# lcp29/trimesh-ray-optix

Hardware: AMD Instinct MI355X
Metric: Mrays/s closest-hit, 1M-tri mesh, 1024^2 ray batch (higher is better)
Workload: dtype f32; 1 GPU; C5(i): icosphere(8)+displacement seed 0, 1310720 tris; 1024x1024 pinhole rays per GPU; intersects_closest (stream_compaction=False); rays_per_gpu=1048576, rays_total=1048576, triangles=1310720, parallelism=ray-sharded x1, BVH replicated, warmup_steps_done=352, bvh_depth=30, bvh_bytes=104857568

## Files before the change

### trimesh-ray-optix_amd/csrc/kernels_direct.inc

```
template <bool C, bool DEEP = false> struct tr_word { typedef uint64_t T; };
template <> struct tr_word<true, false> { typedef uint32_t T; };

constexpr bool TR_STREAM_QN = true;
template <int Q> constexpr bool TR_STREAM_COLD = Q != TR_Q_CLOSEST;
template <int Q, int K, bool STATS, bool COMPACT = false, bool UNI = false, bool DEEP = false>
__device__ __forceinline__ void wave_traverse(const tr_bvh_view& b, tr_ray& r, bool go,
                                              tr_result& res, tr_topk<K>& top, tr_counters* cnt,
                                              const tr_ring ring) {
    tr_result_init(res);
    if (Q == TR_Q_LOCATION) top.init();
    typedef typename tr_word<COMPACT, DEEP>::T W;
    tr_state_t<W> fs;
    tr_state_init(fs);
    if (!go) fs.node = -1;
    while (!tr_done(fs)) {
        tr_fused_step<Q, K, STATS, COMPACT, W, UNI, true>(b, r, fs, res, top, cnt, ring);
        TR_CONVERGE();
        tr_fused_step<Q, K, STATS, COMPACT, W, UNI, false>(b, r, fs, res, top, cnt, ring);
        TR_CONVERGE();
    }
}

constexpr uint32_t TR_STEAL_EVERY = 3u;
constexpr uint32_t TR_STEAL_EARLY = 4u;
constexpr int TR_STEAL_IDLE = 1;
__device__ __forceinline__ int lane_rank(unsigned long long mask) {
    return (int)__builtin_amdgcn_mbcnt_hi((unsigned)(mask >> 32), __builtin_amdgcn_mbcnt_lo((unsigned)mask, 0u));
}

template <int Q, bool STATS, bool COMPACT, bool DEEP = false, bool QN = false>
__device__ __forceinline__ bool wave_traverse_steal(const tr_bvh_view& b, tr_ray& r, bool go,
                                                    tr_result& res, tr_counters* cnt,
                                                    const tr_ring ring, int32_t* wl, int lane,
                                                    uint32_t steal_min, bool& lost) {
    constexpr bool PLAIN = QN;
    typedef typename std::conditional<PLAIN, tr_plaina_w, typename tr_word<COMPACT, DEEP>::T>::type W;
    lost = false;
    tr_result_init(res);
    tr_topk<1> top;
    tr_state_t<W> fs;
    const tr_aring ar = tr_aring_of(ring);
    (void)ar;
    if constexpr (PLAIN) tr_state_init(fs, tr_addr_start(ring));
    else tr_state_init(fs);
    if (!go) fs.node = -1;
    auto trip_step = [&](auto test_tag) {
        constexpr bool TEST = decltype(test_tag)::value;
        if (!tr_done(fs)) tr_fused_step<Q, 1, STATS, COMPACT, W, false, TEST, QN>(b, r, fs, res, top, cnt, ring);
    };
    int owner = lane;
    bool split = false;
    uint32_t trip = 0;
    if (steal_min & 0x8000u) {
        steal_min &= 0x7fffu;
        const unsigned long long act = __ballot(go);
        if (act != 0ull) {
            const int l0 = (int)__builtin_ctzll(act);
            const float ax = __shfl(r.dx, l0), ay = __shfl(r.dy, l0), az = __shfl(r.dz, l0);
            const float bx = __shfl(r.ox, l0) - r.ox, by = __shfl(r.oy, l0) - r.oy, bz = __shfl(r.oz, l0) - r.oz;
            const float dd = ax * r.dx + ay * r.dy + az * r.dz;
            const float n0 = ax * ax + ay * ay + az * az, n1 = r.dx * r.dx + r.dy * r.dy + r.dz * r.dz;
            const float ex = 65535.f * b.frame.scale[0], ey = 65535.f * b.frame.scale[1], ez = 65535.f * b.frame.scale[2];
            const bool alike = dd > 0.f && dd * dd >= 0.998f * n0 * n1 && bx * bx + by * by + bz * bz <= 1e-4f * (ex * ex + ey * ey + ez * ez);
            if (4 * __popcll(__ballot(go && alike)) < 3 * __popcll(act) && steal_min > TR_STEAL_EARLY) steal_min = TR_STEAL_EARLY;
        }
    }
    typedef __attribute__((address_space(3))) volatile int32_t lds_i32;
    typedef __attribute__((address_space(3))) volatile unsigned long long lds_u64;
    lds_i32* const lw = (lds_i32*)wl;
    lds_i32* const list = lw;
    lds_i32* const xnode = lw + 64;
    lds_i32* const xdepth = lw + 128;
    int32_t* const xflags = wl + 128;
    if constexpr (PLAIN) xdepth[lane] = 0;
    constexpr int ACC = 192;
    int32_t* sum = wl + ACC;
    unsigned long long* keys = reinterpret_cast<unsigned long long*>(wl + ACC);
    lds_i32* const vsum = lw + ACC;
    lds_u64* const vkeys = (lds_u64*)(lw + ACC);
    lds_i32* const vslots = lw + ACC + 128;
    auto deposit = [&]() {
        if constexpr (PLAIN) {
            if (tr_addr_lost(fs.sa)) atomicOr(&xflags[owner], 0x100);
        }
        if (Q == TR_Q_COUNT) {
            if (res.count) atomicAdd(&sum[owner], res.count);
        } else if (Q == TR_Q_ANY) {
            if (res.best_face >= 0) vsum[owner] = 1;
        } else {
            const bool have = res.best_slot >= 0;
            const unsigned long long key = ((unsigned long long)(__float_as_uint(res.best_t) & 0x7fffffffu) << 32) |
                                           (unsigned)res.best_face;
            if (have) atomicMin(&keys[owner], key);
            __builtin_amdgcn_wave_barrier();
            if (have && vkeys[owner] == key) vslots[owner] = res.best_slot;
        }
    };
    for (;;) {
#pragma unroll 1
        for (uint32_t k = 0; k <= TR_STEAL_EVERY; k += 2) {
            trip_step(std::true_type{});
            TR_CONVERGE();
            trip_step(std::false_type{});
            TR_CONVERGE();
        }
        trip += (TR_STEAL_EVERY / 2u + 1u) * 2u;
        if (split) {
            if (Q == TR_Q_ANY) {
                if (res.best_face >= 0) vsum[owner] = 1;
                __builtin_amdgcn_wave_barrier();
                if (vsum[owner] != 0 && !tr_done(fs)) { fs.node = -1; fs.p0 = -1; fs.p1 = -1; fs.p2 = -1; }
            } else if (Q == TR_Q_CLOSEST || Q == TR_Q_FIRST) {
                const bool have = res.best_slot >= 0;
                const unsigned long long mine = ((unsigned long long)(__float_as_uint(res.best_t) & 0x7fffffffu) << 32) |
                                                (unsigned)(res.best_face < 0 ? 0x7fffffff : res.best_face);
                if (have) atomicMin(&keys[owner], mine);
                __builtin_amdgcn_wave_barrier();
                const unsigned long long k = vkeys[owner];
                if (have && k == mine) vslots[owner] = res.best_slot;
                if (k < mine) {
                    tr_set_best_t(res, __uint_as_float((unsigned)(k >> 32)));
                    res.best_face = (int32_t)(unsigned)k;
                    res.best_slot = -1;
                }
            }
        }
        const bool done = tr_done(fs);
        const unsigned long long idle = __ballot(done);
        if (idle == ~0ull) break;
        if (__popcll(idle) >= TR_STEAL_IDLE && trip >= steal_min) {
            uint32_t bot = 0;
            bool has_far;
            if constexpr (PLAIN) {
                bot = (uint32_t)xdepth[lane] & 0xffu;
                has_far = tr_addr_can_give(ar, fs.sa, bot);
            } else {
                has_far = (fs.trail & fs.owned) != 0;
            }
            const bool can_give = !done && has_far;
            const unsigned long long donors = __ballot(can_give);
            const int ni = __popcll(idle), nd = __popcll(donors);
            const int np = ni < nd ? ni : nd;
            if (np > 0) {
                if (!split) {
                    if (Q == TR_Q_COUNT || Q == TR_Q_ANY) vsum[lane] = 0;
                    else vkeys[lane] = ~0ull;
                    split = true;
                    __builtin_amdgcn_wave_barrier();
                }
                const int drank = lane_rank(donors), irank = lane_rank(idle);
                const bool give = can_give && drank < np;
                int gnode = 0, gdepth = 0;
                (void)gdepth;
                if constexpr (PLAIN) {
                    if (give) {
                        gnode = tr_addr_give(ar, fs.sa, bot);
                        list[drank] = lane; xnode[lane] = gnode;
                        atomicAdd(&xflags[lane], 1);
                    }
                } else if (give) {
                    uint32_t j;
                    gnode = tr_ring_get(ring, tr_bottom_slot<W>(fs.trail, fs.owned, j));
                    gdepth = (int32_t)(j + 1);
                    list[drank] = lane; xnode[lane] = gnode; xdepth[lane] = gdepth;
                    fs.trail &= ~(W(1) << j);
                }
                __builtin_amdgcn_wave_barrier();
                const bool take = done && irank < np;
                const int src = take ? list[irank] : lane;
                if (take) {
                    deposit();
                    tr_result_init(res);
                }
                r.ox = __shfl(r.ox, src); r.oy = __shfl(r.oy, src); r.oz = __shfl(r.oz, src);
                r.dx = __shfl(r.dx, src); r.dy = __shfl(r.dy, src); r.dz = __shfl(r.dz, src);
                r.ix = __shfl(r.ix, src); r.iy = __shfl(r.iy, src); r.iz = __shfl(r.iz, src);
                r.kd = __shfl(r.kd, src);
                r.sel_n = (uint32_t)__shfl((int)r.sel_n, src); r.sel_f = (uint32_t)__shfl((int)r.sel_f, src); r.sel_z = (uint32_t)__shfl((int)r.sel_z, src);
                if constexpr (QN) {
                    r.qax = __shfl(r.qax, src); r.qay = __shfl(r.qay, src); r.qaz = __shfl(r.qaz, src);
                    r.qnx = __shfl(r.qnx, src); r.qny = __shfl(r.qny, src); r.qnz = __shfl(r.qnz, src);
                    r.qfx = __shfl(r.qfx, src); r.qfy = __shfl(r.qfy, src); r.qfz = __shfl(r.qfz, src);
                    r.qaz2 = r.qaz;
                }
                const int own2 = __shfl(owner, src);
                const float bt = __shfl(res.best_t, src);
                if (take) {
                    owner = own2;
                    if constexpr (PLAIN) {
                        tr_state_init(fs, tr_addr_bottom(ar, fs.sa));
                        atomicAnd(&xflags[lane], 0x100);
                    } else {
                        tr_state_init(fs);
                        fs.depth = (uint32_t)xdepth[src];
                    }
                    fs.node = xnode[src];
                    tr_set_best_t(res, bt);
                }
                __builtin_amdgcn_wave_barrier();
            }
        }
    }
    if (split) {
        deposit();
        __builtin_amdgcn_wave_barrier();
        if (Q == TR_Q_COUNT) {
            res.count = vsum[lane];
        } else if (Q == TR_Q_ANY) {
            res.best_face = vsum[lane] ? 0 : -1;
        } else {
            const unsigned long long k = vkeys[lane];
            tr_result_init(res);
            if (k != ~0ull) {
                tr_set_best_t(res, __uint_as_float((unsigned)(k >> 32)));
                res.best_face = (int32_t)(unsigned)k;
                res.best_slot = vslots[lane];
            }
        }
        if constexpr (PLAIN) lost = (xdepth[lane] & 0x100) != 0;
    } else if constexpr (PLAIN) {
        lost = tr_addr_lost(fs.sa);
    }
    return split;
}

template <int Q, bool STATS, bool COMPACT = false, bool UNI = false, bool DEEP = false>
__device__ __forceinline__ void process_ray(const tr_bvh_view& b, const RayFetch& rf,
                                            const QueryOut& out, int64_t i, bool in_range,
                                            tr_counters* cnt, const tr_ring ring) {
    float o[3] = {0.f, 0.f, 0.f}, d[3] = {0.f, 0.f, 0.f};
    if (in_range) fetch_ray(rf, i, o, d);
    tr_ray r;
    const bool valid = tr_ray_setup_a(r, b.frame, o[0], o[1], o[2], d[0], d[1], d[2]) && in_range;
    tr_result res;
    if (Q == TR_Q_LOCATION) {
        tr_topk<0> top;
        top.ent = out.hits + (in_range ? i : 0) * out.cap;
        top.tris = b.tris;
        top.cap = out.cap;
        if (b.num_tris >= 2) {
            wave_traverse<Q, 0, STATS, COMPACT, UNI, DEEP>(b, r, valid, res, top, cnt, ring);
        } else {
            top.init();
            brute_one<Q>(b, r, valid, res);
            if (res.count) top.insert(res.best_t, res.best_face, 0);
        }
    } else {
        tr_topk<1> top;
        if (b.num_tris >= 2) wave_traverse<Q, 1, STATS, COMPACT, UNI, DEEP>(b, r, valid, res, top, cnt, ring);
        else brute_one<Q>(b, r, valid, res);
    }
    if (in_range) write_result<Q>(b, out, i, r, res);
}

template <int Q>
__device__ __attribute__((noinline)) tr_result retraverse_lost(const tr_node* nodes, const tr_link* links, const tr_tri* tris,
                                                               float b0, float b1, float b2, float s0, float s1, float s2,
                                                               float ox, float oy, float oz, float dx, float dy, float dz,
                                                               float best_t, int32_t best_face, int32_t best_slot) {
    tr_bvh_view v;
    v.nodes = nodes; v.links = links; v.tris = tris; v.num_tris = 2; v.qnodes = nullptr; v.frame_dev = nullptr;
    v.frame.base[0] = b0; v.frame.base[1] = b1; v.frame.base[2] = b2;
    v.frame.scale[0] = s0; v.frame.scale[1] = s1; v.frame.scale[2] = s2;
    tr_result res;
    res.best_t = best_t; res.best_face = best_face; res.best_slot = best_slot; res.count = 0;
    tr_ray r;
    if (tr_ray_setup_a(r, v.frame, ox, oy, oz, dx, dy, dz)) {
        tr_topk<1> top;
        tr_counters* nc = nullptr;
        tr_traverse_more<Q, 1, false>(v, r, res, top, nc);
    }
    return res;
}

template <int Q, bool STATS, bool COMPACT, bool DEEP = false, bool QN = false>
__device__ __forceinline__ void process_ray_steal(const tr_bvh_view& b, const RayFetch& rf,
                                                  const QueryOut& out, int64_t i, bool in_range,
                                                  tr_counters* cnt, const tr_ring ring, int32_t* wl,
                                                  uint32_t steal_min) {
    float o[3] = {0.f, 0.f, 0.f}, d[3] = {0.f, 0.f, 0.f};
    if (in_range) fetch_ray(rf, i, o, d);
    tr_ray r;
    const bool valid = tr_ray_setup_q(r, b.frame, o[0], o[1], o[2], d[0], d[1], d[2]) && in_range;
    tr_result res;
    bool split = false, lost = false;
    if (b.num_tris >= 2) split = wave_traverse_steal<Q, STATS, COMPACT, DEEP, QN>(b, r, valid, res, cnt, ring, wl, (int)(threadIdx.x & 63), steal_min, lost);
    else brute_one<Q>(b, r, valid, res);
    if (split && in_range) {
        fetch_ray(rf, i, o, d);
        tr_ray_setup_a(r, b.frame, o[0], o[1], o[2], d[0], d[1], d[2]);
    }
    if constexpr (QN) {
        lost = lost && valid;
        if (__builtin_expect(TR_WAVE_ANY(lost), 0)) {
            if (lost) {
                fetch_ray(rf, i, o, d);
                res = retraverse_lost<Q>(b.nodes, b.links, b.tris, b.frame.base[0], b.frame.base[1], b.frame.base[2],
                                         b.frame.scale[0], b.frame.scale[1], b.frame.scale[2], o[0], o[1], o[2], d[0], d[1], d[2],
                                         res.best_t, res.best_face, res.best_slot);
            }
        }
    }
    if (in_range) write_result<Q>(b, out, i, r, res);
}

template <int Q, int K, bool STATS, bool COMPACT, bool DEEP = false>
__device__ __forceinline__ void wave_traverse_unordered(const tr_bvh_view& b, tr_ray& r, bool go,
                                                        tr_result& res, tr_topk<K>& top, tr_counters* cnt,
                                                        const tr_ring ring, const tr_leafq lq, int leaf_min) {
    typedef typename tr_word<COMPACT, DEEP>::T W;
    tr_result_init(res);
    if (Q == TR_Q_LOCATION) top.init();
    tr_ustate_t<W> st;
    tr_ustate_init(st);
    if (!go) st.node = -1;
    for (;;) {
        const bool can_node = tr_ucan_node(st);
        const unsigned long long mn = __ballot(can_node), ml = __ballot(st.nq > 0);
        if ((mn | ml) == 0ull) break;
        const bool parked = st.node >= 0 && !can_node;
        const bool leaf_phase = mn == 0ull || __ballot(parked) != 0ull || (int)__popcll(ml) >= (int)leaf_min;
        tr_unord_step<Q, K, STATS, COMPACT, W>(b, r, can_node, leaf_phase, st, res, top, cnt, ring, lq);
        TR_CONVERGE();
    }
}

template <int Q, bool STATS, bool COMPACT, bool DEEP = false>
__device__ __forceinline__ int wave_count_unordered_steal(const tr_bvh_view& b, tr_ray& r, bool go, tr_counters* cnt,
                                                          const tr_ring ring, const tr_leafq lq, int leaf_min,
                                                          int lane, uint32_t steal_min) {
    typedef typename tr_word<COMPACT, DEEP>::T W;
    tr_result res;
    tr_result_init(res);
    tr_topk<1> top;
    tr_ustate_t<W> st;
    tr_ustate_init(st);
    if (!go) st.node = -1;
    int owner = lane;
    int acc = 0;
    uint32_t trip = 0;
    auto hand_in = [&](bool want) {
        unsigned long long m = __ballot(want && res.count != 0);
        while (m != 0ull) {
            const int t = (int)__builtin_ctzll(m);
            const int o = __builtin_amdgcn_readlane(owner, t), c = __builtin_amdgcn_readlane(res.count, t);
            if (lane == o) acc += c;
            m &= m - 1ull;
        }
        if (want) res.count = 0;
    };
    for (;;) {
        bool live = true;
#pragma unroll 1
        for (int k = 0; k < 4 && live; k++) {
            const bool can_node = tr_ucan_node(st);
            const unsigned long long mn = __ballot(can_node), ml = __ballot(st.nq > 0);
            live = (mn | ml) != 0ull;
            if (live) {
                const bool parked = st.node >= 0 && !can_node;
                const bool leaf_phase = mn == 0ull || __ballot(parked) != 0ull || (int)__popcll(ml) >= (int)leaf_min;
                tr_unord_step<Q, 1, STATS, COMPACT, W>(b, r, can_node, leaf_phase, st, res, top, cnt, ring, lq);
            }
            TR_CONVERGE();
        }
        trip += 4;
        const bool done = tr_udone(st);
        const unsigned long long idle = __ballot(done);
        if (idle == ~0ull) break;
        if (idle == 0ull) continue;
        const W cand = st.trail & st.owned;
        const bool can_give = !done && cand != 0 && trip >= steal_min;
        const unsigned long long donors = __ballot(can_give);
        const int ni = __popcll(idle), nd = __popcll(donors);
        const int np = ni < nd ? ni : nd;
        if (np == 0) continue;
        const int drank = lane_rank(donors), irank = lane_rank(idle);
        const bool give = can_give && drank < np;
        const bool take = done && irank < np;
        const unsigned long long givers = __ballot(give);
        const int tgt = give ? drank : 63 - lane_rank(~givers);
        const int list = __builtin_amdgcn_ds_permute(tgt << 2, lane);
        const int pick = __shfl(list, irank & 63);
        const int src = take ? pick : lane;
        int gnode = 0, gdepth = 0;
        if (give) {
            const uint32_t j = (uint32_t)__builtin_ctzll((unsigned long long)cand);
            gnode = tr_ring_get(ring, j & (TR_RING - 1));
            gdepth = (int)(j + 1);
            st.trail &= ~(W(1) << j);
            st.owned &= ~(W(1) << j);
        }
        if (take && owner == lane) { acc += res.count; res.count = 0; }
        hand_in(take && owner != lane);
        r.ox = __shfl(r.ox, src); r.oy = __shfl(r.oy, src); r.oz = __shfl(r.oz, src);
        r.dx = __shfl(r.dx, src); r.dy = __shfl(r.dy, src); r.dz = __shfl(r.dz, src);
        r.ix = __shfl(r.ix, src); r.iy = __shfl(r.iy, src); r.iz = __shfl(r.iz, src);
        r.kd = __shfl(r.kd, src);
        r.sel_n = (uint32_t)__shfl((int)r.sel_n, src); r.sel_f = (uint32_t)__shfl((int)r.sel_f, src); r.sel_z = (uint32_t)__shfl((int)r.sel_z, src);
        r.qax = __shfl(r.qax, src); r.qay = __shfl(r.qay, src); r.qaz = __shfl(r.qaz, src);
        r.qnx = __shfl(r.qnx, src); r.qny = __shfl(r.qny, src); r.qnz = __shfl(r.qnz, src);
        r.qfx = __shfl(r.qfx, src); r.qfy = __shfl(r.qfy, src); r.qfz = __shfl(r.qfz, src);
        r.qaz2 = r.qaz;
        const int own2 = __shfl(owner, src), n2 = __shfl(gnode, src), d2 = __shfl(gdepth, src);
        if (take) {
            owner = own2;
            tr_ustate_init(st);
            st.node = n2;
            st.depth = (uint32_t)d2;
// ... 384 lines not shown
```

### trimesh-ray-optix_amd/csrc/tr_bvh.h

```cpp
#pragma once
#include <type_traits>
#include "tr_math.h"
#include "../../include/triro_hip.h"

struct alignas(16) tr_f4 {
    float x, y, z, w;
};
struct alignas(16) tr_i4 {
    int32_t x, y, z, w;
};

struct alignas(64) tr_node {
    float box0[6];
    float box1[6];
    int32_t c0, c1;
    int32_t parent;
    int32_t sibling;
};
static_assert(sizeof(tr_node) == 64, "node must be 64 B");
TR_HD void tr_node_set_box(float* box, const float* lo, const float* hi) {
    box[0] = lo[0]; box[1] = lo[1]; box[2] = lo[2]; box[3] = hi[2]; box[4] = hi[0]; box[5] = hi[1];
}

struct alignas(8) tr_link {
// ... 492 lines not shown
    if (STATS) cnt->nodes++;
    float tn0, tf0, tn1, tf1;
    tr_node_slabs(r, n0, n1, n2, tn0, tf0, tn1, tf1);
    union { float f; int32_t i; } u0, u1, u2, u3;
    u0.f = n3.x; u1.f = n3.y; u2.f = n3.z; u3.f = n3.w;
    const int32_t c0 = u0.i, c1 = u1.i;
    int32_t parent = u2.i, sibling = u3.i;
    const float lim = tr_cull_limit<Q>(res);
    bool h0 = tr_slab_hit(tn0, tf0, lim);
    bool h1 = tr_slab_hit(tn1, tf1, lim);
    if (h0 && c0 < 0) { st.p0 = ~c0; h0 = false; }
    if (h1 && c1 < 0) { st.p1 = ~c1; h1 = false; }
    if (h0 | h1) {
        const bool both = h0 & h1;
        const bool swap = both ? (tn1 < tn0) : h1;
        if (both) {
            tr_push_far(ring, st.trail, st.owned, st.depth, swap ? c0 : c1);
            st.trail |= (1ull << st.depth);
        }
        st.node = swap ? c1 : c0;
        st.depth++;
    } else if (st.trail == 0) {
        st.node = -1;
    } else {
        uint32_t j = 0;
        int32_t far = -1;
        if (tr_pop_far(ring, st.trail, st.owned, j, far)) {
            st.node = far;
        } else {
            int32_t node = st.node;
            uint32_t depth = st.depth;
            while (depth > j + 1) {
                node = parent;
                const tr_link l = b.links[node];
                parent = l.parent; sibling = l.sibling;
                depth--;
                if (STATS) cnt->climbs++;
            }
            st.node = sibling;
        }
        st.depth = j + 1;
    }
}

template <int Q, int K, bool STATS>
TR_HD void tr_leaf_step(const tr_bvh_view& b, const tr_ray& r, tr_state& st, tr_result& res,
                        tr_topk<K>& top, tr_counters* cnt) {
    const int32_t q0 = st.p0, q1 = st.p1;
    tr_counters* nc = nullptr;
    const bool any1 = TR_WAVE_ANY(q1 >= 0);
    const tr_tri t0 = tr_load_tri<false>(b, q0 >= 0 ? q0 : 0, nc);
    tr_tri t1 = t0;
    if (any1) t1 = tr_load_tri<false>(b, q1 >= 0 ? q1 : 0, nc);
    if (STATS && q0 >= 0) cnt->tris++;
    bool fin = tr_fold_leaf<Q, K>(q0 >= 0, r, t0, q0, res, top, st.pe);
    fin = tr_drain_exact<Q, K>(b, r, st.pe, res, top) || fin;
    if (any1) {
        const bool live = q1 >= 0 && !fin;
        if (STATS && live) cnt->tris++;
        fin = tr_fold_leaf<Q, K>(live, r, t1, q1, res, top, st.pe) || fin;
        fin = tr_drain_exact<Q, K>(b, r, st.pe, res, top) || fin;
    }
    st.p0 = -1; st.p1 = -1;
    if (Q == TR_Q_ANY && fin) st.node = -1;
}

TR_HD void tr_qnode_slabs_contract(const tr_ray& r, const tr_qframe& f, const tr_i4& w0, const tr_i4& w1,
                                   float& tn0, float& tf0, float& tn1, float& tf1) {
    const uint32_t q0 = (uint32_t)w0.x, q1 = (uint32_t)w0.y, q2 = (uint32_t)w0.z, q3 = (uint32_t)w0.w;
    const uint32_t q4 = (uint32_t)w1.x, q5 = (uint32_t)w1.y;
    const float sx = f.scale[0], sy = f.scale[1], sz = f.scale[2], bx = f.base[0], by = f.base[1], bz = f.base[2];
    tr_slab(r, tr_qdecode(q0 & 0xffffu, sx, bx), tr_qdecode(q0 >> 16, sy, by), tr_qdecode(q1 & 0xffffu, sz, bz),
            tr_qdecode(q2 & 0xffffu, sx, bx), tr_qdecode(q2 >> 16, sy, by), tr_qdecode(q1 >> 16, sz, bz), tn0, tf0);
    tr_slab(r, tr_qdecode(q3 & 0xffffu, sx, bx), tr_qdecode(q3 >> 16, sy, by), tr_qdecode(q4 & 0xffffu, sz, bz),
            tr_qdecode(q5 & 0xffffu, sx, bx), tr_qdecode(q5 >> 16, sy, by), tr_qdecode(q4 >> 16, sz, bz), tn1, tf1);
}

TR_HD void tr_qnode_slabs(const tr_ray& r, const tr_qframe& f, const tr_i4& w0, const tr_i4& w1,
                          float& tn0, float& tf0, float& tn1, float& tf1) {
#if defined(__HIP_DEVICE_COMPILE__)
    const uint32_t q0 = (uint32_t)w0.x, q1 = (uint32_t)w0.y, q2 = (uint32_t)w0.z, q3 = (uint32_t)w0.w;
    const uint32_t q4 = (uint32_t)w1.x, q5 = (uint32_t)w1.y;
    typedef float tr_v2 __attribute__((ext_vector_type(2)));
    const tr_v2 axy = {r.qax, r.qay}, azz = {r.qaz, r.qaz2};
    const tr_v2 nxy = {r.qnx, r.qny}, fxy = {r.qfx, r.qfy}, bz = {r.qnz, r.qfz};
#define TR_UNPK(w) tr_v2{(float)((w) & 0xffffu), (float)((w) >> 16)}
    {
        const uint32_t pn = __builtin_amdgcn_perm(q2, q0, r.sel_n), pf = __builtin_amdgcn_perm(q2, q0, r.sel_f);
        const uint32_t zz = __builtin_amdgcn_perm(q1, q1, r.sel_z);
        const tr_v2 a = __builtin_elementwise_fma(TR_UNPK(pn), axy, nxy);
        const tr_v2 c = __builtin_elementwise_fma(TR_UNPK(pf), axy, fxy);
        const tr_v2 b = __builtin_elementwise_fma(TR_UNPK(zz), azz, bz);
        tn0 = fmaxf(fmaxf(a.x, a.y), b.x);
        tf0 = fminf(fminf(c.x, c.y), b.y);
    }
    {
        const uint32_t pn = __builtin_amdgcn_perm(q5, q3, r.sel_n), pf = __builtin_amdgcn_perm(q5, q3, r.sel_f);
        const uint32_t zz = __builtin_amdgcn_perm(q4, q4, r.sel_z);
        const tr_v2 a = __builtin_elementwise_fma(TR_UNPK(pn), axy, nxy);
        const tr_v2 c = __builtin_elementwise_fma(TR_UNPK(pf), axy, fxy);
        const tr_v2 b = __builtin_elementwise_fma(TR_UNPK(zz), azz, bz);
        tn1 = fmaxf(fmaxf(a.x, a.y), b.x);
        tf1 = fminf(fminf(c.x, c.y), b.y);
    }
#undef TR_UNPK
#else
    (void)f;
    const bool nx = r.ix < 0.f, ny = r.iy < 0.f, nz = r.iz < 0.f;
    const uint32_t q[6] = {(uint32_t)w0.x, (uint32_t)w0.y, (uint32_t)w0.z, (uint32_t)w0.w, (uint32_t)w1.x, (uint32_t)w1.y};
    float tn[2], tf[2];
    for (int c = 0; c < 2; c++) {
        const uint32_t lox = q[3 * c] & 0xffffu, loy = q[3 * c] >> 16, loz = q[3 * c + 1] & 0xffffu;
        const uint32_t hiz = q[3 * c + 1] >> 16, hix = q[3 * c + 2] & 0xffffu, hiy = q[3 * c + 2] >> 16;
        const float ax = fmaf((float)(nx ? hix : lox), r.qax, r.qnx), ay = fmaf((float)(ny ? hiy : loy), r.qay, r.qny);
        const float az = fmaf((float)(nz ? hiz : loz), r.qaz, r.qnz);
        const float cx = fmaf((float)(nx ? lox : hix), r.qax, r.qfx), cy = fmaf((float)(ny ? loy : hiy), r.qay, r.qfy);
        const float cz = fmaf((float)(nz ? loz : hiz), r.qaz, r.qfz);
        tn[c] = fmaxf(fmaxf(ax, ay), az);
        tf[c] = fminf(fminf(cx, cy), cz);
    }
    tn0 = tn[0]; tf0 = tf[0]; tn1 = tn[1]; tf1 = tf[1];
#endif
}

template <bool STATS>
TR_HD int32_t tr_climb(const tr_bvh_view& b, int32_t node, uint32_t depth, uint32_t j, tr_counters* cnt) {
    tr_link l = b.links[node];
    if (STATS) cnt->climbs++;
    while (depth > j + 1) {
        node = l.parent;
        l = b.links[node];
        depth--;
        if (STATS) cnt->climbs++;
    }
    return l.sibling;
}

struct tr_rec_f { tr_f4 n0, n1, n2, n3; };
struct tr_rec_q { tr_i4 w0, w1; };
TR_HD void tr_rec_slabs(const tr_bvh_view&, const tr_ray& r, const tr_rec_f& n, float& tn0, float& tf0, float& tn1, float& tf1) {
    tr_node_slabs(r, n.n0, n.n1, n.n2, tn0, tf0, tn1, tf1);
}
TR_HD void tr_rec_slabs(const tr_bvh_view& b, const tr_ray& r, const tr_rec_q& n, float& tn0, float& tf0, float& tn1, float& tf1) {
    tr_qnode_slabs(r, b.frame, n.w0, n.w1, tn0, tf0, tn1, tf1);
}
TR_HD void tr_rec_children(const tr_rec_f& n, int32_t& c0, int32_t& c1) {
    union { float f; int32_t i; } u0, u1;
    u0.f = n.n3.x; u1.f = n.n3.y; c0 = u0.i; c1 = u1.i;
}
TR_HD void tr_rec_children(const tr_rec_q& n, int32_t& c0, int32_t& c1) { c0 = n.w1.z; c1 = n.w1.w; }
TR_HD void tr_rec_links(const tr_rec_f& n, int32_t& parent, int32_t& sibling) {
    union { float f; int32_t i; } u2, u3;
    u2.f = n.n3.z; u3.f = n.n3.w; parent = u2.i; sibling = u3.i;
}
TR_HD void tr_rec_links(const tr_rec_q&, int32_t& parent, int32_t& sibling) { parent = -1; sibling = -1; }

template <int Q, int K, bool STATS, bool COMPACT, typename W, bool TEST, bool COLD, typename REC>
TR_HD void tr_fused_body(const tr_bvh_view& b, const tr_ray& r, tr_state_t<W>& st, tr_result& res,
                         tr_topk<K>& top, tr_counters* cnt, const tr_ring ring, const bool has_node,
                         const REC& rec) {
    if (STATS && has_node) cnt->nodes++;
    bool fin = false;
    const int32_t q0 = st.p0;
    if (TEST && TR_WAVE_ANY(q0 >= 0)) {
        tr_counters* nc = nullptr;
        const tr_tri t0 = tr_load_tri<false, COMPACT>(b, q0 >= 0 ? q0 : 0, nc);
        const bool live = q0 >= 0;
        if (STATS && live) cnt->tris++;
        fin = tr_fold_leaf<Q, K>(live, r, t0, q0, res, top, st.pe);
    }
    if (Q == TR_Q_ANY && fin) { st.node = -1; st.p1 = -1; st.p2 = -1; }
    float tn0, tf0, tn1, tf1;
    tr_rec_slabs(b, r, rec, tn0, tf0, tn1, tf1);
    int32_t c0, c1, parent, sibling;
    tr_rec_children(rec, c0, c1);
    tr_rec_links(rec, parent, sibling);
    const float lim = tr_cull_limit<Q>(res);
    const bool go = has_node && st.node >= 0;
    bool h0 = tr_slab_hit(tn0, tf0, lim) && go;
    bool h1 = tr_slab_hit(tn1, tf1, lim) && go;
    if (!TEST) {
        const bool l0 = h0 && c0 < 0, l1 = h1 && c1 < 0;
        h0 = h0 && c0 >= 0;
        h1 = h1 && c1 >= 0;
        if (go) {
            const bool hb = st.p0 >= 0, two = l0 && l1;
            const int32_t xi = l0 ? ~c0 : (l1 ? ~c1 : -1);
            st.p2 = (hb && two) ? ~c1 : -1;
            st.p1 = hb ? xi : (two ? ~c1 : -1);
            st.p0 = hb ? st.p0 : xi;
        }
    } else {
        const bool l0 = h0 && c0 < 0;
        const bool wait = st.p2 >= 0;
        const bool l1 = (h1 && c1 < 0) || wait;
        h0 = h0 && c0 >= 0;
        h1 = h1 && c1 >= 0;
        const int32_t i1 = wait ? st.p2 : ~c1;
        const bool hb = st.p1 >= 0, two = l0 && l1;
        const int32_t xi = l0 ? ~c0 : (l1 ? i1 : -1);
        st.p0 = hb ? st.p1 : xi;
        st.p1 = hb ? xi : (two ? i1 : -1);
        st.p2 = (hb && two) ? i1 : -1;
    }
    if constexpr (std::is_same<W, tr_plain_w>::value) {
        if (go) {
            const bool both = h0 && h1;
            const bool swap = (both && tn1 < tn0) || !h0;
            if (both) tr_plain_push(ring, st.sp, swap ? c0 : c1);
            st.node = swap ? c1 : c0;
            if (!(h0 || h1)) st.node = tr_plain_pop(ring, st.sp);
        }
    } else if constexpr (std::is_same<W, tr_plaina_w>::value) {
        if (go) {
            const tr_aring ar = tr_aring_of(ring);
            const bool both = h0 && h1;
            const bool swap = (both && tn1 < tn0) || !h0;
            if (both) tr_addr_push(ar, st.sa, swap ? c0 : c1);
            st.node = swap ? c1 : c0;
            if (!(h0 || h1)) st.node = tr_addr_pop(ar, st.sa);
        }
    } else if (go) {
        if (h0 || h1) {
            const bool both = h0 && h1;
            const bool swap = (both && tn1 < tn0) || !h0;
            if (both) {
                tr_push_far(ring, st.trail, st.owned, st.depth, swap ? c0 : c1);
                st.trail |= (W(1) << st.depth);
            }
            st.node = swap ? c1 : c0;
            st.depth++;
        } else if (st.trail == 0) {
            st.node = -1;
        } else {
            uint32_t j = 0;
            int32_t far = -1;
            if (!tr_pop_far(ring, st.trail, st.owned, j, far)) {
                if constexpr (std::is_same<REC, tr_rec_f>::value) {
                    int32_t node = st.node;
                    uint32_t depth = st.depth;
                    while (depth > j + 1) {
                        node = parent;
                        const tr_link l = b.links[node];
                        parent = l.parent; sibling = l.sibling;
                        depth--;
                        if (STATS) cnt->climbs++;
                    }
                    far = sibling;
                } else {
                    far = tr_climb<STATS>(b, st.node, st.depth, j, cnt);
                }
            }
            st.node = far;
            st.depth = j + 1;
        }
    }
    if (TEST) {
        if (tr_drain_exact<Q, K, COMPACT, COLD>(b, r, st.pe, res, top) && Q == TR_Q_ANY) { st.node = -1; st.p0 = -1; st.p1 = -1; st.p2 = -1; }
        st.pe = -1;
    }
}


template <int Q, int K, bool STATS, bool COMPACT = false, typename W = uint64_t, bool UNI = false, bool TEST = true,
          bool QN = false, bool COLD = true>
TR_HD void tr_fused_step(const tr_bvh_view& b, const tr_ray& r, tr_state_t<W>& st, tr_result& res,
                         tr_topk<K>& top, tr_counters* cnt, const tr_ring ring) {
    const int32_t room = TEST ? st.p2 : st.p1;
    const bool has_node = st.node >= 0 && room < 0;
#if defined(__HIP_DEVICE_COMPILE__)
    if (UNI) {
        const unsigned long long m = __ballot(has_node);
        if (m != 0ull) {
            const int32_t nu = __builtin_amdgcn_readlane(st.node, (int)__builtin_ctzll(m));
            if (__ballot(has_node && st.node != nu) == 0ull) {
                if constexpr (QN) {
                    typedef const __attribute__((address_space(4))) tr_i4* tr_ci4p;
                    const tr_ci4p sp = (tr_ci4p)(unsigned long long)tr_qnode_ptr<COMPACT>(b, nu);
                    const tr_rec_q rec = {sp[0], sp[1]};
                    tr_fused_body<Q, K, STATS, COMPACT, W, TEST, COLD>(b, r, st, res, top, cnt, ring, has_node, rec);
                } else {
                    typedef const __attribute__((address_space(4))) tr_f4* tr_cf4p;
                    const tr_cf4p sp = (tr_cf4p)(unsigned long long)tr_node_ptr<COMPACT>(b, nu);
                    const tr_rec_f rec = {sp[0], sp[1], sp[2], sp[3]};
                    tr_fused_body<Q, K, STATS, COMPACT, W, TEST, COLD>(b, r, st, res, top, cnt, ring, has_node, rec);
                }
                return;
            }
        }
    }
#endif
    const int32_t nidx = st.node & ~(st.node >> 31) & (room >> 31);
    if constexpr (QN) {
        const tr_i4* np = tr_qnode_ptr<COMPACT>(b, nidx);
        const tr_rec_q rec = {np[0], np[1]};
        tr_fused_body<Q, K, STATS, COMPACT, W, TEST, COLD>(b, r, st, res, top, cnt, ring, has_node, rec);
    } else {
        const tr_f4* np = tr_node_ptr<COMPACT>(b, nidx);
        const tr_rec_f rec = {np[0], np[1], np[2], np[3]};
        tr_fused_body<Q, K, STATS, COMPACT, W, TEST, COLD>(b, r, st, res, top, cnt, ring, has_node, rec);
    }
}


constexpr int TR_LEAFQ = 6;
struct tr_leafq {
    int32_t* base;
    int32_t stride;
};

template <typename W>
struct tr_ustate_t {
    int32_t node;
    uint32_t depth;
    W trail, owned;
    int32_t nq;
    int32_t pe;
};

template <typename W>
TR_HD void tr_ustate_init(tr_ustate_t<W>& st) { st.node = 0; st.depth = 0; st.trail = 0; st.owned = 0; st.nq = 0; st.pe = -1; }
template <typename W>
TR_HD bool tr_udone(const tr_ustate_t<W>& st) { return st.node < 0 && st.nq == 0 && st.pe < 0; }
template <typename W>
TR_HD bool tr_ucan_node(const tr_ustate_t<W>& st) { return st.node >= 0 && st.nq <= TR_LEAFQ - 2; }

template <int Q, int K, bool STATS, bool COMPACT, typename W>
TR_HD void tr_unord_step(const tr_bvh_view& b, const tr_ray& r, bool go_node, bool leaf_phase,
                         tr_ustate_t<W>& st, tr_result& res, tr_topk<K>& top, tr_counters* cnt,
                         const tr_ring ring, const tr_leafq lq) {
    const int32_t nidx = go_node ? st.node : 0;
    const tr_i4* np = COMPACT ? reinterpret_cast<const tr_i4*>(reinterpret_cast<const char*>(b.qnodes) + ((uint32_t)nidx << 5))
                              : reinterpret_cast<const tr_i4*>(b.qnodes + nidx);
    const tr_i4 w0 = np[0], w1 = np[1];
    if (STATS && go_node) cnt->nodes++;
    bool fin = false;
    if (leaf_phase) {
        const bool gl = st.nq > 0;
        int32_t slot = 0;
        if (gl) { st.nq--; slot = lq.base[st.nq * lq.stride]; }
        tr_counters* nc = nullptr;
        const tr_tri t = tr_load_tri<false, COMPACT>(b, slot, nc);
        if (STATS && gl) cnt->tris++;
        fin = tr_fold_leaf<Q, K>(gl, r, t, slot, res, top, st.pe);
    }
    if (Q == TR_Q_ANY && fin) { st.node = -1; st.nq = 0; }
    const bool go = go_node && !fin;
    float tn0, tf0, tn1, tf1;
    tr_qnode_slabs(r, b.frame, w0, w1, tn0, tf0, tn1, tf1);
    const int32_t c0 = w1.z, c1 = w1.w;
    bool h0 = tr_slab_hit(tn0, tf0, TR_TLIM) && go;
    bool h1 = tr_slab_hit(tn1, tf1, TR_TLIM) && go;
    if (h0 && c0 < 0) { lq.base[st.nq * lq.stride] = ~c0; st.nq++; h0 = false; }
    if (h1 && c1 < 0) { lq.base[st.nq * lq.stride] = ~c1; st.nq++; h1 = false; }
    if (go) {
        if (h0 || h1) {
            const bool both = h0 && h1;
            const bool swap = (Q == TR_Q_ANY) ? ((both && tn1 < tn0) || !h0) : !h0;
            if (both) {
                st.trail |= (W(1) << st.depth);
                if (ring.base) {
                    const uint32_t slot = st.depth & (TR_RING - 1);
                    tr_ring_put(ring, slot, swap ? c0 : c1);
                    st.owned = (st.owned & ~(tr_ring_mask(W(0)) << slot)) | (W(1) << st.depth);
                }
            }
            st.node = swap ? c1 : c0;
            st.depth++;
        } else if (st.trail == 0) {
            st.node = -1;
        } else {
            const uint32_t j = tr_top_bit(st.trail);
            st.trail &= ~(W(1) << j);
            if (ring.base && ((st.owned >> j) & W(1))) st.node = tr_ring_get(ring, j & (TR_RING - 1));
            else st.node = tr_climb<STATS>(b, st.node, st.depth, j, cnt);
            st.depth = j + 1;
        }
    }
    if (leaf_phase) {
        if (tr_drain_exact<Q, K, COMPACT>(b, r, st.pe, res, top) && Q == TR_Q_ANY) { st.node = -1; st.nq = 0; }
        st.pe = -1;
    }
}

template <int Q, int K, bool STATS>
TR_HD void tr_traverse_unordered(const tr_bvh_view& b, const tr_ray& r, bool valid, tr_result& res,
                                 tr_topk<K>& top, tr_counters* cnt, const tr_ring ring, const tr_leafq lq) {
    tr_result_init(res);
    if (Q == TR_Q_LOCATION) top.init();
    if (!valid || b.num_tris < 2) return;
    tr_ustate_t<uint64_t> st;
    tr_ustate_init(st);
    while (!tr_udone(st)) {
        const bool cn = tr_ucan_node(st);
        tr_unord_step<Q, K, STATS, false, uint64_t>(b, r, cn, !cn, st, res, top, cnt, ring, lq);
        TR_CONVERGE();
    }
}

template <int Q, int K, bool STATS>
TR_HD void tr_traverse_more(const tr_bvh_view& b, const tr_ray& r, tr_result& res, tr_topk<K>& top, tr_counters* cnt) {
    if (Q == TR_Q_ANY && res.best_face >= 0) return;
    tr_state st;
    tr_state_init(st);
    while (!tr_done(st)) {
        if (tr_pending(st)) tr_leaf_step<Q, K, STATS>(b, r, st, res, top, cnt);
        else tr_node_step<Q, STATS>(b, r, st, res, cnt, tr_ring{nullptr, 0});
        TR_CONVERGE();
    }
}

template <int Q, int K, bool STATS>
TR_HD void tr_traverse(const tr_bvh_view& b, const tr_ray& r, bool valid, tr_result& res,
                       tr_topk<K>& top, tr_counters* cnt, const tr_ring ring = tr_ring{nullptr, 0}) {
    tr_result_init(res);
    if (Q == TR_Q_LOCATION) top.init();
    if (!valid || b.num_tris < 2) return;
    tr_state st;
    tr_state_init(st);
    while (!tr_done(st)) {
        if (tr_pending(st)) tr_leaf_step<Q, K, STATS>(b, r, st, res, top, cnt);
        else tr_node_step<Q, STATS>(b, r, st, res, cnt, ring);
        TR_CONVERGE();
    }
}
```

Baseline: 7749 Mrays/s.

## Add leaf-free descent prologue before fused traversal loop in plain path

Adds a specialized descent-only step that traverses internal BVH nodes without leaf intersection code. It runs at the start of the PLAIN work-stealing kernel until any lane in the wave reaches a leaf, then hands the pending leaves to the fused loop and realigns the trip counter with the steal cadence. The aim is to cut the per-step cost of the early, leaf-free levels of a deep BVH. It adds extra wave votes, a parity fixup and more code complexity. The steal-cadence bookkeeping could also be subtly wrong.

After: 7904 Mrays/s (median of 6 runs). 1.02x the previous value.

```diff
diff --git a/trimesh-ray-optix_amd/csrc/kernels_direct.inc b/trimesh-ray-optix_amd/csrc/kernels_direct.inc
--- a/trimesh-ray-optix_amd/csrc/kernels_direct.inc
+++ b/trimesh-ray-optix_amd/csrc/kernels_direct.inc
@@ -96,14 +96,36 @@
             if (have && vkeys[owner] == key) vslots[owner] = res.best_slot;
         }
     };
+    uint32_t k0 = 0;
+    if constexpr (PLAIN) {
+        bool l0 = false, l1 = false;
+        int32_t c0 = 0, c1 = 0;
+        while (trip < steal_min) {
+            l0 = false; l1 = false;
+            if (fs.node >= 0) tr_descent_step<Q, STATS, COMPACT>(b, r, fs, res, cnt, ring, l0, l1, c0, c1);
+            TR_CONVERGE();
+            trip++;
+            if (TR_WAVE_ANY(l0 || l1) || !TR_WAVE_ANY(fs.node >= 0)) break;
+        }
+        fs.p0 = l0 ? ~c0 : (l1 ? ~c1 : -1);
+        fs.p1 = (l0 && l1) ? ~c1 : -1;
+        if (trip & 1u) {
+            trip_step(std::false_type{});
+            TR_CONVERGE();
+            trip++;
+        }
+        k0 = trip == 0u ? 0u : ((trip - 1u) & TR_STEAL_EVERY) + 1u;
+        trip -= k0;
+    }
     for (;;) {
 #pragma unroll 1
-        for (uint32_t k = 0; k <= TR_STEAL_EVERY; k += 2) {
+        for (uint32_t k = k0; k <= TR_STEAL_EVERY; k += 2) {
             trip_step(std::true_type{});
             TR_CONVERGE();
             trip_step(std::false_type{});
             TR_CONVERGE();
         }
+        k0 = 0;
         trip += (TR_STEAL_EVERY / 2u + 1u) * 2u;
         if (split) {
             if (Q == TR_Q_ANY) {
diff --git a/trimesh-ray-optix_amd/csrc/tr_bvh.h b/trimesh-ray-optix_amd/csrc/tr_bvh.h
--- a/trimesh-ray-optix_amd/csrc/tr_bvh.h
+++ b/trimesh-ray-optix_amd/csrc/tr_bvh.h
@@ -818,6 +818,30 @@
     }
 }
 
+template <int Q, bool STATS, bool COMPACT>
+TR_HD void tr_descent_step(const tr_bvh_view& b, const tr_ray& r, tr_astate& st, const tr_result& res, tr_counters* cnt,
+                           const tr_ring ring, bool& l0, bool& l1, int32_t& c0, int32_t& c1) {
+    const tr_i4* np = tr_qnode_ptr<COMPACT>(b, st.node);
+    const tr_rec_q rec = {np[0], np[1]};
+    if (STATS) cnt->nodes++;
+    float tn0, tf0, tn1, tf1;
+    tr_rec_slabs(b, r, rec, tn0, tf0, tn1, tf1);
+    tr_rec_children(rec, c0, c1);
+    const float lim = tr_cull_limit<Q>(res);
+    bool h0 = tr_slab_hit(tn0, tf0, lim);
+    bool h1 = tr_slab_hit(tn1, tf1, lim);
+    l0 = h0 && c0 < 0;
+    l1 = h1 && c1 < 0;
+    h0 = h0 && c0 >= 0;
+    h1 = h1 && c1 >= 0;
+    const tr_aring ar = tr_aring_of(ring);
+    const bool both = h0 && h1;
+    const bool swap = (both && tn1 < tn0) || !h0;
+    if (both) tr_addr_push(ar, st.sa, swap ? c0 : c1);
+    st.node = swap ? c1 : c0;
+    if (!(h0 || h1)) st.node = tr_addr_pop(ar, st.sa);
+}
+
 
 constexpr int TR_LEAFQ = 6;
 struct tr_leafq {
```
